# pmgbergen/porepy

Hardware: AMD Instinct MI355X
Metric: cells/sec MPFA assemble+solve, 3D unstructured grid (higher is better)
Workload: dtype f64

## Files before the change

### include/porefv.h

```cpp
#ifndef POREFV_H
#define POREFV_H

#include <stddef.h>
#include <stdint.h>

#ifdef __cplusplus
extern "C" {
#endif

typedef struct pfv_ctx pfv_ctx;

typedef enum {
  PFV_OK = 0,
  PFV_ERR_SINGULAR = 1,
  PFV_ERR_CELL_SHAPE = 2,
  PFV_ERR_HIP = 3,
  PFV_ERR_ARGUMENT = 4,
  PFV_ERR_UNSUPPORTED = 5,
  PFV_ERR_NOT_CONVERGED = 6
} pfv_status;

enum {
  PFV_MAT_FLUX = 0,
  PFV_MAT_BOUND_FLUX = 1,
// ... 128 lines not shown
  double flow_adjoint_map_ms;
  double flow_adjoint_products_ms;
  double flow_adjoint_solve_ms;
  double flow_adjoint_gradient_ms;
  double advdiff_adjoint_ms;
  int64_t advdiff_adjoint_steps;
  int64_t advdiff_adjoint_iterations;
  int64_t advdiff_adjoint_gmres_retries;
  int64_t advdiff_adjoint_precond_fallbacks;
  double advdiff_adjoint_accumulate_ms;
  int64_t flow_adjoint_exact_calls;
  int64_t flow_adjoint_exact_map_builds;
  double flow_adjoint_exact_map_ms;
  double flow_adjoint_exact_ms;
  int64_t spgemm_path;
  int64_t spgemm_lds_bytes;
  double advdiff_adjoint_exact_ms;
  int64_t advdiff_adjoint_exact_passes;
  int64_t advdiff_adjoint_exact_batch;
  double transport_sorb_ms;
  int64_t transport_sorb_steps;
  int64_t transport_sorb_core_iterations;
  int64_t transport_sorb_components;
} pfv_stats;

pfv_status pfv_create(int device, pfv_ctx** out);
void pfv_destroy(pfv_ctx* h);
const char* pfv_last_error(pfv_ctx* h);
int pfv_is_device_build(void);

pfv_status pfv_set_grid(pfv_ctx* h, int nd, int64_t nc, int64_t nf, int64_t nn,
                        const double* nodes, const int32_t* cf_indptr,
                        const int32_t* cf_indices, const int8_t* cf_sign,
                        const int32_t* fn_indptr, const int32_t* fn_indices,
                        const double* face_normals, const double* face_centers,
                        const double* cell_centers, const double* face_areas);

pfv_status pfv_mpfa_set_params(pfv_ctx* h, const double* perm_33n, const uint8_t* bc_flags,
                               const double* robin_weight, double eta,
                               const double* eta_subface);

pfv_status pfv_mpfa_set_permeability(pfv_ctx* h, const double* perm_33n);

#define PFV_AD_WANT_FLUX_JACOBIAN 1u
pfv_status pfv_mpfa_ad_flux_system(pfv_ctx* h, const double* p, const double* dk_dp, const double* bc_values,
                                   const double* vector_source, const double* source, double* flux_out,
// ... 235 lines not shown
pfv_status pfv_csr_divide(pfv_csr* A, double s);
pfv_status pfv_csr_spmv(const pfv_csr* A, const double* x, double* y);
pfv_status pfv_csr_spmv_device(const pfv_csr* A, const double* d_x, double* d_y);
pfv_status pfv_csr_info(const pfv_csr* A, int64_t* nrows, int64_t* ncols, int64_t* nnz);
pfv_status pfv_csr_get(const pfv_csr* A, int32_t* indptr, int32_t* indices, double* values);
pfv_status pfv_csr_set_system(pfv_ctx* h, const pfv_csr* A, const double* rhs, int rhs_on_device);
void pfv_csr_free(pfv_csr* A);

pfv_status pfv_set_stream(pfv_ctx* h, void* hip_stream);
pfv_status pfv_reset_stream(pfv_ctx* h);
pfv_status pfv_sync(pfv_ctx* h);

pfv_status pfv_get_stats(pfv_ctx* h, pfv_stats* out);
pfv_status pfv_get_stats_n(pfv_ctx* h, void* out, size_t struct_size);

enum { PFV_KERNEL_SPMV_A = 0, PFV_KERNEL_NODE = 1, PFV_KERNEL_FACE = 2,
       PFV_KERNEL_AMG_SMOOTH = 3,
       PFV_KERNEL_TRIAD = 4,
       PFV_KERNEL_READ = 5         };
pfv_status pfv_time_kernel(pfv_ctx* h, int kernel, int reps, double* avg_ms);

pfv_status pfv_debug_copy(pfv_ctx* h, int which, double* dst, int64_t count);

#ifdef __cplusplus
}
#endif
#endif
```

### porepy_amd/_lib.py

```python
from __future__ import annotations

import ctypes as C
import os

import numpy as np

_HERE = os.path.dirname(os.path.abspath(__file__))
DEFAULT_LIBRARY = os.path.join(_HERE, "csrc", "libporefv_hip.so")

MAT_FLUX, MAT_BOUND_FLUX, MAT_BOUND_PRESSURE_CELL, MAT_BOUND_PRESSURE_FACE = 0, 1, 2, 3
MAT_VECTOR_SOURCE, MAT_BOUND_PRESSURE_VECTOR_SOURCE, MAT_SYSTEM = 4, 5, 6
MAT_STRESS, MAT_BOUND_STRESS, MAT_BOUND_DISPLACEMENT_CELL, MAT_BOUND_DISPLACEMENT_FACE, MAT_MECH_SYSTEM = 7, 8, 9, 10, 11
MAT_USER_SYSTEM = 12
MAT_FLUX_JACOBIAN = 13
MAT_UPWIND, MAT_UPWIND_RHS_DIR, MAT_UPWIND_RHS_NEU, MAT_TRANSPORT_SYSTEM = 14, 15, 16, 17
MAT_ADVDIFF_SYSTEM = 18
BC_DIR, BC_NEU, BC_ROB, BC_INTERNAL = 1, 2, 4, 8
SOLVE_CG, SOLVE_BICGSTAB, SOLVE_GMRES = 0, 1, 2
PRECOND_JACOBI, PRECOND_AMG, PRECOND_BLOCK, PRECOND_AMG_NNS, PRECOND_SWEEP = 0, 1, 2, 3, 4
FLUXFN_LINEAR, FLUXFN_COREY, FLUXFN_TABLE = 0, 1, 2
ISOTHERM_LINEAR, ISOTHERM_FREUNDLICH, ISOTHERM_LANGMUIR = 0, 1, 2
DISCR_REBUILD_TOPOLOGY, DISCR_SKIP_VECTOR_SOURCE = 1, 2

STATUS_NAMES = {
# ... 2 lines not shown
}

EXPORTS = [
    "pfv_create", "pfv_destroy", "pfv_last_error", "pfv_is_device_build", "pfv_set_grid",
    "pfv_mpfa_set_params", "pfv_mpfa_discretize", "pfv_matrix_info", "pfv_get_matrix",
    "pfv_mpfa_assemble", "pfv_get_rhs", "pfv_spmv", "pfv_solve", "pfv_spmv_device",
    "pfv_get_device_rhs", "pfv_sync", "pfv_get_stats", "pfv_time_kernel", "pfv_debug_copy",
    "pfv_spmv_device_rows", "pfv_copy_device_vector", "pfv_set_stream",
    "pfv_mpsa_set_params", "pfv_mpsa_discretize", "pfv_mpsa_assemble",
    "pfv_mpfa_discretize_faces", "pfv_set_system", "pfv_tpfa_discretize", "pfv_mpsa_discretize_faces", "pfv_set_preconditioner", "pfv_amg_setup", "pfv_amg_setup_sharded", "pfv_amg_apply_device", "pfv_csr_from_host", "pfv_csr_from_matrix", "pfv_csr_block_diag", "pfv_csr_matmul", "pfv_csr_axpby", "pfv_csr_transpose", "pfv_csr_bmat", "pfv_csr_scale", "pfv_csr_divide", "pfv_csr_spmv", "pfv_csr_spmv_device", "pfv_csr_info", "pfv_csr_get", "pfv_csr_set_system", "pfv_csr_free", "pfv_reset_stream", "pfv_mpsa_set_robin", "pfv_mpsa_set_basis", "pfv_mpfa_set_subface_bc", "pfv_mpsa_set_subface_bc", "pfv_mpsa_set_subface_basis",
    "pfv_biot_set_alphas", "pfv_biot_discretize", "pfv_biot_matrix_info", "pfv_biot_get_matrix",
    "pfv_set_vectors_on_device", "pfv_set_periodic", "pfv_biot_discretize_faces", "pfv_solve_sharded", "pfv_tpfa_transmissibility_ad",
    "pfv_get_matrix_rows", "pfv_active_size", "pfv_device_memory",
    "pfv_rccl_unique_id", "pfv_rccl_comm_create", "pfv_rccl_set_halo_plan", "pfv_rccl_hooks", "pfv_rccl_stats",
    "pfv_rccl_last_error", "pfv_rccl_comm_destroy", "pfv_mpfa_ad_flux_system", "pfv_host_alloc", "pfv_host_free",
    "pfv_mpsa_set_subface_eta", "pfv_mpsa_set_reconstruction_eta", "pfv_mpsa_set_reconstruction_eta_subface", "pfv_get_stats_n", "pfv_set_block_preconditioner",
    "pfv_mpfa_set_permeability", "pfv_set_near_null_space", "pfv_amg_nns_level", "pfv_amg_nns_apply_device", "pfv_amg_level",
    "pfv_mpfa_face_flux", "pfv_upwind_set_bc", "pfv_upwind_discretize", "pfv_upwind_assemble", "pfv_transport_advance",
    "pfv_advdiff_assemble", "pfv_advdiff_advance", "pfv_advdiff_face_flux", "pfv_resident_flux",
    "pfv_sweep_info", "pfv_transport_advance_multi", "pfv_transport_advance_nl", "pfv_transport_advance_nl_multi",
    "pfv_transport_advance_react", "pfv_transport_adjoint_multi", "pfv_transport_adjoint_react",
    "pfv_transport_adjoint_nl", "pfv_transport_adjoint_nl_multi", "pfv_flow_adjoint", "pfv_flow_adjoint_exact",
    "pfv_advdiff_adjoint", "pfv_advdiff_adjoint_exact", "pfv_amg_level_rhs", "pfv_transport_advance_sorb",
]


class SolveInfo(C.Structure):
    _fields_ = [("iterations", C.c_int32), ("converged", C.c_int32),
                ("rel_residual", C.c_double), ("solve_ms", C.c_double)]


class Stats(C.Structure):
    _fields_ = [("topology_ms", C.c_double), ("symbolic_ms", C.c_double), ("node_ms", C.c_double),
                ("face_ms", C.c_double), ("assemble_ms", C.c_double), ("solve_ms", C.c_double),
                ("bytes_written_outputs", C.c_double), ("num_nodes", C.c_int64),
                ("num_sub_half_faces", C.c_int64), ("sum_block_sq", C.c_int64),
                ("max_block", C.c_int64), ("amg_setup_ms", C.c_double),
                ("amg_operator_complexity", C.c_double), ("amg_levels", C.c_int64),
                ("amg_coarsest_rows", C.c_int64), ("discretize_ms", C.c_double), ("solve_renumbered", C.c_int64),
                ("node_flops", C.c_double), ("node_table_doubles", C.c_int64),
                ("amg_maps_reused", C.c_int64), ("amg_level0_nnz", C.c_int64), ("amg_filter_theta", C.c_double),
                ("win_reused", C.c_int64), ("amg_filter_layout", C.c_int64),
                ("solve_launches", C.c_int64), ("amg_setup_launches", C.c_int64), ("node_redo", C.c_int64),
                ("symbolic_reused", C.c_int64), ("amg_stale_rematches", C.c_int64),
                ("mpsa_contrast_regions", C.c_int64), ("mpsa_max_contrast", C.c_double), ("assemble_positions_kept", C.c_int64),
                ("pipeline_runs", C.c_int64), ("amg_nns_modes", C.c_int64),
# ... 13 lines not shown
                ("transport_react_ms", C.c_double), ("transport_react_steps", C.c_int64),
                ("transport_react_core_iterations", C.c_int64), ("transport_react_components", C.c_int64),
                ("transport_adjoint_ms", C.c_double), ("transport_adjoint_steps", C.c_int64),
                ("transport_adjoint_core_iterations", C.c_int64), ("amg_ap_nnz", C.c_int64),
                ("transport_react_adjoint_ms", C.c_double), ("transport_react_adjoint_steps", C.c_int64),
                ("transport_react_adjoint_core_iterations", C.c_int64), ("amg_galerkin_ap", C.c_int64),
                ("transport_nl_adjoint_ms", C.c_double), ("transport_nl_adjoint_steps", C.c_int64),
                ("transport_nl_adjoint_core_iterations", C.c_int64),
                ("transport_nlc_adjoint_ms", C.c_double), ("transport_nlc_adjoint_steps", C.c_int64),
                ("transport_nlc_adjoint_core_iterations", C.c_int64),
                ("flow_adjoint_calls", C.c_int64), ("flow_adjoint_iterations", C.c_int64),
                ("flow_adjoint_map_builds", C.c_int64), ("flow_adjoint_map_ms", C.c_double),
                ("flow_adjoint_products_ms", C.c_double), ("flow_adjoint_solve_ms", C.c_double),
                ("flow_adjoint_gradient_ms", C.c_double),
                ("advdiff_adjoint_ms", C.c_double), ("advdiff_adjoint_steps", C.c_int64),
                ("advdiff_adjoint_iterations", C.c_int64), ("advdiff_adjoint_gmres_retries", C.c_int64),
                ("advdiff_adjoint_precond_fallbacks", C.c_int64), ("advdiff_adjoint_accumulate_ms", C.c_double),
                ("flow_adjoint_exact_calls", C.c_int64), ("flow_adjoint_exact_map_builds", C.c_int64),
                ("flow_adjoint_exact_map_ms", C.c_double), ("flow_adjoint_exact_ms", C.c_double),
                ("spgemm_path", C.c_int64), ("spgemm_lds_bytes", C.c_int64),
                ("advdiff_adjoint_exact_ms", C.c_double), ("advdiff_adjoint_exact_passes", C.c_int64),
                ("advdiff_adjoint_exact_batch", C.c_int64),
                ("transport_sorb_ms", C.c_double), ("transport_sorb_steps", C.c_int64),
                ("transport_sorb_core_iterations", C.c_int64), ("transport_sorb_components", C.c_int64)]

    def as_dict(self):
        return {n: getattr(self, n) for n, _ in self._fields_}


HALO_FN = C.CFUNCTYPE(C.c_int, C.c_void_p, C.c_void_p, C.c_void_p)
ALLREDUCE_FN = C.CFUNCTYPE(C.c_int, C.c_void_p, C.c_void_p, C.c_int, C.c_void_p)


SENDRECV_FN = C.CFUNCTYPE(C.c_int, C.c_void_p, C.c_int, C.POINTER(C.c_int32), C.c_void_p, C.POINTER(C.c_int64),
                          C.c_void_p, C.POINTER(C.c_int64), C.c_void_p)
ALLGATHER_FN = C.CFUNCTYPE(C.c_int, C.c_void_p, C.c_void_p, C.c_void_p, C.c_int64, C.c_void_p)


class ShardHooks(C.Structure):
    _fields_ = [("exchange_halo", HALO_FN), ("allreduce_sum", ALLREDUCE_FN), ("user", C.c_void_p),
                ("sendrecv", SENDRECV_FN), ("allgather", ALLGATHER_FN)]


class PorefvError(RuntimeError):
    def __init__(self, status: int, message: str):
        super().__init__(f"porefv status {status} ({STATUS_NAMES.get(status, '?')}): {message}")
        self.status = status
# ... 141 lines not shown
    lib.pfv_rccl_comm_create.restype = C.c_int
    lib.pfv_rccl_set_halo_plan.argtypes = [C.c_void_p, C.c_int, _ip, _i64p, _ip, _i64p, _ip]
    lib.pfv_rccl_set_halo_plan.restype = C.c_int
    lib.pfv_rccl_hooks.argtypes = [C.c_void_p, C.POINTER(ShardHooks)]
    lib.pfv_rccl_hooks.restype = C.c_int
    lib.pfv_rccl_stats.argtypes = [C.c_void_p, _i64p, _i64p, _i64p]
    lib.pfv_rccl_stats.restype = C.c_int
    lib.pfv_rccl_last_error.argtypes = [C.c_void_p]
    lib.pfv_rccl_last_error.restype = C.c_char_p
    lib.pfv_rccl_comm_destroy.argtypes = [C.c_void_p]
    lib.pfv_rccl_comm_destroy.restype = None
    lib.pfv_device_memory.argtypes = [_h, C.POINTER(C.c_int64), C.POINTER(C.c_int64)]
    lib.pfv_device_memory.restype = C.c_int
    lib.pfv_host_alloc.argtypes = [C.c_size_t, C.POINTER(C.c_void_p)]
    lib.pfv_host_alloc.restype = C.c_int
    lib.pfv_host_free.argtypes = [C.c_void_p]
    lib.pfv_host_free.restype = None
    lib.pfv_active_size.argtypes = [_h, C.POINTER(C.c_int64)]
    lib.pfv_active_size.restype = C.c_int
    lib.pfv_get_matrix_rows.argtypes = [_h, C.c_int, C.c_int64, _ip, _ip, _ip, _dp]
    lib.pfv_get_matrix_rows.restype = C.c_int
    lib.pfv_debug_copy.argtypes = [_h, C.c_int, _dp, C.c_int64]
    lib.pfv_debug_copy.restype = C.c_int
    lib.pfv_spmv_device_rows.argtypes = [_h, C.c_int, C.c_int64, C.c_void_p, C.c_void_p]
    lib.pfv_spmv_device_rows.restype = C.c_int
    lib.pfv_copy_device_vector.argtypes = [_h, C.c_int, C.c_void_p, C.c_int64]
    lib.pfv_copy_device_vector.restype = C.c_int
    lib.pfv_tpfa_transmissibility_ad.argtypes = [_h, _dp, _dp, _dp]
    lib.pfv_tpfa_transmissibility_ad.restype = C.c_int
    lib.pfv_solve_sharded.argtypes = [_h, C.c_int, C.c_double, C.c_int, C.c_int64, C.POINTER(ShardHooks),
                                      C.c_void_p, C.c_void_p, C.POINTER(SolveInfo)]
    lib.pfv_solve_sharded.restype = C.c_int
    lib.pfv_set_stream.argtypes = [_h, C.c_void_p]
    lib.pfv_set_stream.restype = C.c_int
    lib.pfv_mpsa_set_params.argtypes = [_h, _dp, _dp, _up, _up, C.c_double]
    lib.pfv_mpsa_set_params.restype = C.c_int
    lib.pfv_mpsa_discretize.argtypes = [_h, C.c_uint32]
    lib.pfv_mpsa_discretize.restype = C.c_int
    lib.pfv_mpsa_assemble.argtypes = [_h, _dp, _dp]
    lib.pfv_mpsa_assemble.restype = C.c_int
    lib.pfv_mpfa_face_flux.argtypes = [_h, _dp, _dp, _dp, _dp]
    lib.pfv_mpfa_face_flux.restype = C.c_int
    lib.pfv_upwind_set_bc.argtypes = [_h, _up]
    lib.pfv_upwind_set_bc.restype = C.c_int
    lib.pfv_upwind_discretize.argtypes = [_h, _dp, C.c_int]
    lib.pfv_upwind_discretize.restype = C.c_int
# ... 1564 lines not shown
               "rel_residual": info.rel_residual, "solve_ms": info.solve_ms}
        return self._adjoint_result(st, grads, out, raise_on_fail)

    def tpfa_transmissibility_ad(self, perm):
        K = _f64(perm)
        if K.shape != (3, 3, self.nc):
            raise ValueError("perm must have shape (3, 3, num_cells)")
        t = np.empty(self.nf, dtype=np.float64)
        jac = np.empty((self.ncf, 9), dtype=np.float64)
        self._check(self.lib.pfv_tpfa_transmissibility_ad(self._h, _ptr(K, _dp), _ptr(t, _dp), _ptr(jac, _dp)))
        return t, jac

    def set_stream(self, stream_ptr: int | None):
        self._check(self.lib.pfv_set_stream(self._h, C.c_void_p(stream_ptr or 0)))

    def reset_stream(self):
        self._check(self.lib.pfv_reset_stream(self._h))

    def debug_array(self, which: int, n: int) -> np.ndarray:
        out = np.empty(n, dtype=np.float64)
        self._check(self.lib.pfv_debug_copy(self._h, int(which), _ptr(out, _dp), n))
        return out

    def time_kernel(self, kernel: int, reps: int = 10) -> float:
        ms = C.c_double()
        self._check(self.lib.pfv_time_kernel(self._h, int(kernel), int(reps), C.byref(ms)))
        return ms.value
```

### porepy_amd/csrc/backend.h

```cpp
#pragma once

#include <algorithm>
#include <atomic>
#include <chrono>
#include <cmath>
#include <cstdint>
#include <cstdio>
#include <cstdlib>
#include <cstring>
#include <numeric>
#include <stdexcept>
#include <string>
#include <type_traits>
#include <unordered_map>
#include <vector>

#ifdef PFV_EMULATE
#define PFV_HD
#define PFV_FN inline
#define PFV_LAMBDA [=]
#else
#include <hip/hip_runtime.h>
#include <rocprim/rocprim.hpp>
#define PFV_HD __host__ __device__
// ... 441 lines not shown
    if (b < n) {
      WaveCtx w{b, pfv_lds + (size_t)grp * lds_per_item, (int)threadIdx.x % G, G, nullptr};
      f(w);
    }
    __syncthreads();
  }
}
#endif

template <class F>
inline void parallel_for(stream_t s, int64_t n, F f) {
  if (n <= 0) return;
#ifdef PFV_EMULATE
  (void)s;
  for (int64_t i = 0; i < n; ++i) f(i);
#else
  int64_t blocks = (n + 255) / 256;
  if (blocks > 16384) blocks = 16384;
  PFV_LAUNCH(HIP_KERNEL_NAME(k_parallel_for<F>), dim3((unsigned)blocks), dim3(256), 0, s, n, f);
  PFV_HIP_CHECK(hipGetLastError());
#endif
}

template <int G = 64, class F>
inline void wave_for(stream_t s, int64_t n, size_t lds_bytes, F f) {
  if (n <= 0) return;
  lds_bytes = (lds_bytes + 15) & ~size_t(15);
#ifdef PFV_EMULATE
  (void)s;
  std::vector<double> lds((lds_bytes + 7) / 8 + 2);
  for (int64_t b = 0; b < n; ++b) {
    WaveCtx w{b, reinterpret_cast<char*>(lds.data()), 0, 1, nullptr};
    f(w);
  }
#else
  constexpr int per_block = 64 / G;
  const size_t block_lds = lds_bytes * per_block;
  if (block_lds > 160 * 1024) throw Error(5, "work item needs more than 160 KiB of LDS");
  int64_t blocks = (n + per_block - 1) / per_block;
  if (blocks > 256 * 64) blocks = 256 * 64;
  if (block_lds > 48 * 1024) {
    PFV_HIP_CHECK(hipFuncSetAttribute(reinterpret_cast<const void*>(&k_wave_for<G, F>),
                                      hipFuncAttributeMaxDynamicSharedMemorySize, (int)block_lds));
  }
  PFV_LAUNCH(HIP_KERNEL_NAME(k_wave_for<G, F>), dim3((unsigned)blocks), dim3(64), block_lds, s, n,
                     lds_bytes, f);
// ... 147 lines not shown

template <class TI, class TO>
inline void exclusive_scan(stream_t s, Scratch& sc, const TI* in, TO* out, size_t n) {
#ifdef PFV_EMULATE
  (void)s; (void)sc;
  TO acc = 0;
  for (size_t i = 0; i < n; ++i) {
    out[i] = acc;
    acc += (TO)in[i];
  }
  out[n] = acc;
#else
  auto it = rocprim::make_transform_iterator(
      rocprim::make_counting_iterator<size_t>(0),
      [in, n] __device__(size_t i) -> TO { return i < n ? (TO)in[i] : TO(0); });
  size_t bytes = 0;
  PFV_HIP_CHECK(rocprim::exclusive_scan(nullptr, bytes, it, out, TO(0), n + 1, rocprim::plus<TO>(), s));
  sc.tmp.ensure(bytes);
  PFV_HIP_CHECK(rocprim::exclusive_scan(sc.tmp.p, bytes, it, out, TO(0), n + 1, rocprim::plus<TO>(), s));
#endif
}

template <class T>
inline T read_scalar(stream_t s, const T* dptr) {
  T v;
  be_d2h(&v, dptr, sizeof(T), s);
  return v;
}

template <class T>
PFV_FN int lower_bound_idx(const T* a, int n, T key) {
  int lo = 0, hi = n;
  while (lo < hi) {
    int mid = (lo + hi) >> 1;
    if (a[mid] < key) lo = mid + 1; else hi = mid;
  }
  return lo;
}

template <class T>
PFV_FN int upper_bound_idx(const T* a, int n, T key) {
  int lo = 0, hi = n;
  while (lo < hi) {
    int mid = (lo + hi) >> 1;
    if (a[mid] <= key) lo = mid + 1; else hi = mid;
  }
// ... 18 lines not shown
}
PFV_HD inline void atomic_max_i32(int* addr, int v) {
#ifdef PFV_EMULATE
  if (v > *addr) *addr = v;
#else
#if defined(__HIP_DEVICE_COMPILE__)
  atomicMax(addr, v);
#else
  (void)addr; (void)v;
#endif
#endif
}
PFV_HD inline void atomic_min_i32(int* addr, int v) {
#ifdef PFV_EMULATE
  if (v < *addr) *addr = v;
#else
#if defined(__HIP_DEVICE_COMPILE__)
  atomicMin(addr, v);
#else
  (void)addr; (void)v;
#endif
#endif
}
PFV_HD inline int atomic_fetch_add_i32(int* addr, int v) {
#ifdef PFV_EMULATE
  const int old = *addr;
  *addr += v;
  return old;
#else
#if defined(__HIP_DEVICE_COMPILE__)
  return atomicAdd(addr, v);
#else
  (void)addr; (void)v;
  return 0;
#endif
#endif
}
PFV_HD inline void atomic_add_i32(int* addr, int v) {
#ifdef PFV_EMULATE
  *addr += v;
#else
#if defined(__HIP_DEVICE_COMPILE__)
  atomicAdd(addr, v);
#else
  (void)addr; (void)v;
#endif
// ... 5 lines not shown
```

### porepy_amd/csrc/ctx.h

```cpp
#pragma once
#include "../../include/porefv.h"
#include "backend.h"

#include <algorithm>
#include <functional>
#include <memory>
#include <vector>

namespace pfv {

constexpr int kMaxFaceNodes = 8;
constexpr int kMaxCellFaces = 16;
constexpr int kMaxBlock = 255;
static const int kClassBounds[] = {4, 8, 12, 16, 24, 32, 40, 48, 64, 96, 128, 192, 255};
constexpr int kNumClasses = 13;

struct alignas(16) SfRec {
  int64_t toff;
  uint8_t n;
  uint8_t ls;
  uint8_t jstar;
  uint8_t deg;
  uint8_t r[3];
  uint8_t pad;
// ... 95 lines not shown
  Buf<int32_t> node_face;
  Buf<int32_t> sf_face;
  Buf<uint8_t> sf_ls;
  Buf<int32_t> face_nsides;
  Buf<int32_t> node_cells;
  Buf<int32_t> node_bptr;
  Buf<int32_t> node_bfaces;
  Buf<uint8_t> node_bls;
  Buf<int64_t> node_tptr;
  Buf<int64_t> node_tbptr;
  Buf<uint8_t> flux_colpairs;
  int64_t cp_stride = 0;
  Buf<uint8_t> node_active;
  Buf<int32_t> face_subset;
  bool biot_rows_complete = false;
  Buf<int32_t> cell_subset;
  Buf<int32_t> face_order;
  double bbox_lo[3] = {0, 0, 0}, bbox_hi[3] = {1, 1, 1};
  Buf<int32_t> node_order;
  std::vector<int64_t> class_begin;
  int max_block = 0, max_deg = 0, max_face_nodes = 0, max_cell_faces = 0, max_bnd_per_node = 0;
  int64_t sum_block_sq = 0;
  int64_t tab_len = 0, tabb_len = 0;

  Buf<double> tab;
  Buf<double> tabb;
  Buf<SfRec> sf_rec;
  Buf<int32_t> face_ctr;
  unsigned face_ctr_next = 0;
  Buf<FaceRec> face_rec;
  Buf<int32_t> status;

  bool have_symbolic = false, have_numeric = false, have_system = false;
  bool have_flow_rhs = false;
  bool rows_complete = false;
  CsrPattern pat_flux, pat_bound, pat_vs, pat_A;
  bool vs_indices_pending = false;
  bool vs_implicit = false;
  Buf<double> val[PFV_NUM_MATS];
  bool filled[PFV_NUM_MATS] = {};
  Buf<double> rhs, diag, xsol, face_tmp, vec_in;
  Buf<double> kry[10];
  Buf<double> red;
  Buf<double> gmres_basis, gmres_small;

  bool have_mpsa_params = false, have_mpsa_numeric = false, have_mpsa_symbolic = false, have_mech_system = false;
// ... 219 lines not shown
```

### porepy_amd/csrc/porefv.hip

```cpp
#include <cmath>
#include <cstring>

#include "ctx.h"
#include "fluxfn.h"
#include "isotherm.h"
#include "react.h"
namespace pfv {
static int rccl_exchange_halo(void* user, double* d_x, void* stream);
}
#include "topology.inc"
#include "mpfa_numeric.inc"
#include "linalg.inc"
#include "reorder.inc"
#include "dd.h"
#include "mpsa.inc"
#include "tpfa.inc"
#include "biot.inc"
#include "ad_flux.inc"
#include "upwind.inc"
#include "advdiff.inc"
#include "sweep.inc"
#include "flow_adjoint.inc"
#include "mpfa_adjoint.inc"
#include "advdiff_adjoint.inc"
// ... 4466 lines not shown
      tm.start(s);
      for (int i = 0; i < reps; ++i) pfv::run_node_kernel(*h);
      *avg_ms = tm.stop(s) / reps;
    } else if (kernel == PFV_KERNEL_FACE) {
      require(h->have_numeric, "discretize first");
      const bool with_vs = h->filled[PFV_MAT_VECTOR_SOURCE];
      tm.start(s);
      for (int i = 0; i < reps; ++i) pfv::run_face_kernel(*h, with_vs);
      *avg_ms = tm.stop(s) / reps;
    } else {
      require(false, "unknown kernel id");
    }
  });
}

pfv_status pfv_debug_copy(pfv_ctx* h, int which, double* dst, int64_t count) {
  return guarded(h, [&] {
    require(h->have_numeric && dst && count >= 0 && count <= (which == 0 ? h->tab_len : h->tabb_len), "bad argument");
    const double* src = which == 0 ? h->tab.p : h->tabb.p;
    be_d2h(dst, src, sizeof(double) * (size_t)count, h->stream);
  });
}

}

#include "rccl_hooks.inc"
#include "csr_algebra.inc"
```

### porepy_amd/csrc/topology.inc

```

namespace pfv {

static void build_topology(pfv_ctx_impl& c) {
  stream_t s = c.stream;
  const int nd = c.nd;
  const int64_t nc = c.nc, nf = c.nf, nn = c.nn, ncf = c.ncf, nsf = c.nsf;
  const int32_t* cf_ptr = c.cf_ptr;
  const int32_t* cf_idx = c.cf_idx;
  const int8_t* cf_sgn = c.cf_sgn;
  const int32_t* fn_ptr = c.fn_ptr;
  const int32_t* fn_idx = c.fn_idx;

  int bits = 1;
  while ((int64_t(1) << bits) < nn + 1 && bits < 32) ++bits;

  Buf<int32_t> cell_of_e, cnt_e;
  Buf<int64_t> h_off;
  cell_of_e.ensure(ncf);
  cnt_e.ensure(ncf + 1);
  h_off.ensure(ncf + 1);
  {
    int32_t* coe = cell_of_e;
    parallel_for(s, nc, PFV_LAMBDA(int64_t cell) {
      for (int e = cf_ptr[cell]; e < cf_ptr[cell + 1]; ++e) coe[e] = (int32_t)cell;
    });
    int32_t* cnt = cnt_e;
// ... 337 lines not shown
      const int n = fp[node + 1] - fp[node];
      int cls = 0;
      while (cls < nclass - 1 && n > bd[cls]) ++cls;
      k[node] = (uint32_t)cls;
      v[node] = (int32_t)node;
    });
    sort_pairs(s, c.scratch, key_in.p, key_out.p, val_in.p, c.node_order.p, (size_t)nn, 4);
    Buf<int32_t> cb_dev;
    int32_t* cbd = cb_dev.ensure(nclass + 1);
    const uint32_t* ks = key_out;
    parallel_for(s, nclass + 1, PFV_LAMBDA(int64_t cls) { cbd[cls] = lower_bound_idx<uint32_t>(ks, (int)nn, (uint32_t)cls); });
    std::vector<int32_t> cbh(nclass + 1);
    be_d2h(cbh.data(), cbd, sizeof(int32_t) * (nclass + 1), s);
    c.class_begin.assign(nclass + 1, nn);
    for (int cls = 0; cls <= nclass; ++cls) c.class_begin[cls] = cbh[cls];
  }
  c.have_topology = true;
  c.topo_key = 0;
  c.stats.num_nodes = nn;
  c.stats.num_sub_half_faces = nh;
  c.stats.sum_block_sq = c.sum_block_sq;
  c.stats.max_block = c.max_block;
  c.stats.node_table_doubles = c.tab_len + c.tabb_len;
}

template <class RankT = uint8_t, int EPL = 4>
PFV_FN int merge_unique_lds(const WaveCtx& w, const int32_t* buf, const int32_t* off, int nl,
                            int32_t* merged, unsigned long long* mask, int32_t* out,
                            RankT* rank_out = nullptr) {
  const int m = off[nl];
  const int nw = (m + 63) >> 6;
  PFV_LANES(i, nw) mask[i] = 0ull;
  for (int e0 = w.lane; e0 < m; e0 += w.width * EPL) {
    int el[EPL], li[EPL], rank[EPL];
    int32_t v[EPL];
#pragma unroll
    for (int u = 0; u < EPL; ++u) {
      const int e = e0 + u * w.width;
      el[u] = e < m ? e : -1;
      const int ee = e < m ? e : 0;
      int l = 0;
      while (l + 1 < nl && ee >= off[l + 1]) ++l;
      li[u] = l;
      v[u] = buf[ee];
      rank[u] = ee - off[l];
    }
// ... 776 lines not shown
```

Measured before the change: 34.77 million.

## Rebuild MPFA topology construction as node-centric pass with fused scans

Adds a new topology builder that constructs per-node sub-half-face tables directly from face-slot arrays. It uses a fused multi-field exclusive scan, per-wave LDS rank sorting, and a single packed device-to-host readback in place of the legacy multi-stage sort pipeline. The aim is to cut kernel launches, global sorts and host syncs during topology setup. If invariants fail (a face with more than two sides, or a node with too many faces), it falls back to the legacy path, which can be forced with an environment variable. A debug export API is also added.

```diff
diff --git a/include/porefv.h b/include/porefv.h
--- a/include/porefv.h
+++ b/include/porefv.h
@@ -174,6 +174,7 @@
   int64_t transport_sorb_steps;
   int64_t transport_sorb_core_iterations;
   int64_t transport_sorb_components;
+  int64_t topology_reference_path;
 } pfv_stats;
 
 pfv_status pfv_create(int device, pfv_ctx** out);
@@ -455,6 +456,8 @@
 
 pfv_status pfv_debug_copy(pfv_ctx* h, int which, double* dst, int64_t count);
 
+pfv_status pfv_debug_topology(pfv_ctx* h, int which, void* dst, int64_t capacity, int64_t* bytes);
+
 #ifdef __cplusplus
 }
 #endif
diff --git a/porepy_amd/_lib.py b/porepy_amd/_lib.py
--- a/porepy_amd/_lib.py
+++ b/porepy_amd/_lib.py
@@ -48,6 +48,7 @@
     "pfv_transport_advance_react", "pfv_transport_adjoint_multi", "pfv_transport_adjoint_react",
     "pfv_transport_adjoint_nl", "pfv_transport_adjoint_nl_multi", "pfv_flow_adjoint", "pfv_flow_adjoint_exact",
     "pfv_advdiff_adjoint", "pfv_advdiff_adjoint_exact", "pfv_amg_level_rhs", "pfv_transport_advance_sorb",
+    "pfv_debug_topology",
 ]
 
 
@@ -107,7 +108,8 @@
                 ("advdiff_adjoint_exact_ms", C.c_double), ("advdiff_adjoint_exact_passes", C.c_int64),
                 ("advdiff_adjoint_exact_batch", C.c_int64),
                 ("transport_sorb_ms", C.c_double), ("transport_sorb_steps", C.c_int64),
-                ("transport_sorb_core_iterations", C.c_int64), ("transport_sorb_components", C.c_int64)]
+                ("transport_sorb_core_iterations", C.c_int64), ("transport_sorb_components", C.c_int64),
+                ("topology_reference_path", C.c_int64)]
 
     def as_dict(self):
         return {n: getattr(self, n) for n, _ in self._fields_}
@@ -295,6 +297,8 @@
     lib.pfv_get_matrix_rows.restype = C.c_int
     lib.pfv_debug_copy.argtypes = [_h, C.c_int, _dp, C.c_int64]
     lib.pfv_debug_copy.restype = C.c_int
+    lib.pfv_debug_topology.argtypes = [_h, C.c_int, C.c_void_p, C.c_int64, _lp]
+    lib.pfv_debug_topology.restype = C.c_int
     lib.pfv_spmv_device_rows.argtypes = [_h, C.c_int, C.c_int64, C.c_void_p, C.c_void_p]
     lib.pfv_spmv_device_rows.restype = C.c_int
     lib.pfv_copy_device_vector.argtypes = [_h, C.c_int, C.c_void_p, C.c_int64]
@@ -1905,6 +1909,31 @@
         self._check(self.lib.pfv_debug_copy(self._h, int(which), _ptr(out, _dp), n))
         return out
 
+    TOPOLOGY_ARRAYS = (
+        ("node_hptr", np.int32), ("h_cell", np.int32), ("h_lf", np.uint8), ("h_sgn", np.int8), ("h_first", np.uint8),
+        ("node_fptr", np.int32), ("node_sf", np.int32), ("sf_face", np.int32), ("sf_ls", np.uint8),
+        ("face_nsides", np.int32), ("node_face", np.int32), ("node_bptr", np.int32), ("node_bfaces", np.int32),
+        ("node_bls", np.uint8), ("node_tptr", np.int64), ("node_tbptr", np.int64), ("node_cells", np.int32),
+        ("face_order", np.int32), ("node_order", np.int32), ("class_begin", np.int64))
+    TOPOLOGY_SCALARS = ("nh", "max_face_nodes", "max_cell_faces", "max_block", "max_deg", "max_bnd_per_node",
+                        "sum_block_sq", "tab_len", "tabb_len", "node_flops_bits", "stats_num_nodes",
+                        "stats_num_sub_half_faces", "stats_sum_block_sq", "stats_max_block",
+                        "stats_node_table_doubles", "topology_digest", "topology_path")
+
+    def debug_topology(self) -> dict:
+        out = {}
+        nbytes = C.c_int64()
+        for which, (name, dtype) in enumerate(self.TOPOLOGY_ARRAYS + (("scalars", np.int64),)):
+            self._check(self.lib.pfv_debug_topology(self._h, which, None, 0, C.byref(nbytes)))
+            arr = np.empty(nbytes.value // np.dtype(dtype).itemsize, dtype=dtype)
+            if arr.size:
+                self._check(self.lib.pfv_debug_topology(self._h, which, arr.ctypes.data_as(C.c_void_p), arr.nbytes,
+                                                        C.byref(nbytes)))
+            out[name] = arr
+        for name, v in zip(self.TOPOLOGY_SCALARS, out.pop("scalars")):
+            out[name] = int(v)
+        return out
+
     def time_kernel(self, kernel: int, reps: int = 10) -> float:
         ms = C.c_double()
         self._check(self.lib.pfv_time_kernel(self._h, int(kernel), int(reps), C.byref(ms)))
diff --git a/porepy_amd/csrc/backend.h b/porepy_amd/csrc/backend.h
--- a/porepy_amd/csrc/backend.h
+++ b/porepy_amd/csrc/backend.h
@@ -487,6 +487,44 @@
 #endif
 }
 
+#ifndef PFV_EMULATE
+template <int NM, class F>
+__global__ void __launch_bounds__(256) k_parallel_for_max(int64_t n, int32_t* out, F f) {
+  __shared__ int32_t red[NM];
+  if ((int)threadIdx.x < NM) red[threadIdx.x] = 0;
+  __syncthreads();
+  int32_t m[NM];
+#pragma unroll
+  for (int k = 0; k < NM; ++k) m[k] = 0;
+  const int64_t stride = (int64_t)gridDim.x * blockDim.x;
+  for (int64_t i = (int64_t)blockIdx.x * blockDim.x + threadIdx.x; i < n; i += stride) f(i, m);
+#pragma unroll
+  for (int k = 0; k < NM; ++k) {
+    if (m[k] > 0) atomicMax(&red[k], m[k]);
+  }
+  __syncthreads();
+  if ((int)threadIdx.x < NM && red[threadIdx.x] > 0) atomicMax(out + threadIdx.x, red[threadIdx.x]);
+}
+#endif
+template <int NM, class F>
+inline void parallel_for_max(stream_t s, int64_t n, int32_t* out, F f) {
+  if (n <= 0) return;
+#ifdef PFV_EMULATE
+  (void)s;
+  int32_t m[NM];
+  for (int k = 0; k < NM; ++k) m[k] = 0;
+  for (int64_t i = 0; i < n; ++i) f(i, m);
+  for (int k = 0; k < NM; ++k) {
+    if (m[k] > out[k]) out[k] = m[k];
+  }
+#else
+  int64_t blocks = (n + 255) / 256;
+  if (blocks > 16384) blocks = 16384;
+  PFV_LAUNCH(HIP_KERNEL_NAME(k_parallel_for_max<NM, F>), dim3((unsigned)blocks), dim3(256), 0, s, n, out, f);
+  PFV_HIP_CHECK(hipGetLastError());
+#endif
+}
+
 template <int G = 64, class F>
 inline void wave_for(stream_t s, int64_t n, size_t lds_bytes, F f) {
   if (n <= 0) return;
@@ -680,6 +718,30 @@
 }
 
 template <class T>
+struct PlusOp {
+  PFV_HD T operator()(const T& a, const T& b) const { return a + b; }
+};
+template <class T, class Gen>
+inline void exclusive_scan_gen(stream_t s, Scratch& sc, Gen gen, T* out, size_t n) {
+#ifdef PFV_EMULATE
+  (void)s; (void)sc;
+  T acc = T();
+  for (size_t i = 0; i < n; ++i) {
+    out[i] = acc;
+    acc = acc + gen((int64_t)i);
+  }
+  out[n] = acc;
+#else
+  auto it = rocprim::make_transform_iterator(rocprim::make_counting_iterator<size_t>(0),
+                                             [gen, n] __device__(size_t i) -> T { return i < n ? gen((int64_t)i) : T(); });
+  size_t bytes = 0;
+  PFV_HIP_CHECK(rocprim::exclusive_scan(nullptr, bytes, it, out, T(), n + 1, PlusOp<T>(), s));
+  sc.tmp.ensure(bytes);
+  PFV_HIP_CHECK(rocprim::exclusive_scan(sc.tmp.p, bytes, it, out, T(), n + 1, PlusOp<T>(), s));
+#endif
+}
+
+template <class T>
 inline T read_scalar(stream_t s, const T* dptr) {
   T v;
   be_d2h(&v, dptr, sizeof(T), s);
@@ -744,6 +806,13 @@
 #endif
 #endif
 }
+PFV_HD inline void store_relaxed_i32(int* addr, int v) {
+#if !defined(PFV_EMULATE) && defined(__HIP_DEVICE_COMPILE__)
+  __hip_atomic_store(addr, v, __ATOMIC_RELAXED, __HIP_MEMORY_SCOPE_AGENT);
+#else
+  *addr = v;
+#endif
+}
 PFV_HD inline int atomic_fetch_add_i32(int* addr, int v) {
 #ifdef PFV_EMULATE
   const int old = *addr;
diff --git a/porepy_amd/csrc/ctx.h b/porepy_amd/csrc/ctx.h
--- a/porepy_amd/csrc/ctx.h
+++ b/porepy_amd/csrc/ctx.h
@@ -141,6 +141,7 @@
   int max_block = 0, max_deg = 0, max_face_nodes = 0, max_cell_faces = 0, max_bnd_per_node = 0;
   int64_t sum_block_sq = 0;
   int64_t tab_len = 0, tabb_len = 0;
+  int topo_path = 0;
 
   Buf<double> tab;
   Buf<double> tabb;
diff --git a/porepy_amd/csrc/porefv.hip b/porepy_amd/csrc/porefv.hip
--- a/porepy_amd/csrc/porefv.hip
+++ b/porepy_amd/csrc/porefv.hip
@@ -4512,6 +4512,59 @@
   });
 }
 
+pfv_status pfv_debug_topology(pfv_ctx* h, int which, void* dst, int64_t capacity, int64_t* bytes) {
+  return guarded(h, [&] {
+    require(h->have_topology && bytes && which >= 0 && which <= 20, "bad argument");
+    auto s = h->stream;
+    const int64_t nn = h->nn, nf = h->nf, nsf = h->nsf, nh = h->nh;
+    const void* src = nullptr;
+    int64_t n = 0;
+    std::vector<int64_t> host;
+    switch (which) {
+      case 0: src = h->node_hptr.p; n = 4 * (nn + 1); break;
+      case 1: src = h->h_cell.p; n = 4 * nh; break;
+      case 2: src = h->h_lf.p; n = nh; break;
+      case 3: src = h->h_sgn.p; n = nh; break;
+      case 4: src = h->h_first.p; n = nh; break;
+      case 5: src = h->node_fptr.p; n = 4 * (nn + 1); break;
+      case 6: src = h->node_sf.p; n = 4 * nsf; break;
+      case 7: src = h->sf_face.p; n = 4 * nsf; break;
+      case 8: src = h->sf_ls.p; n = nsf; break;
+      case 9: src = h->face_nsides.p; n = 4 * nf; break;
+      case 10: src = h->node_face.p; n = 4 * nsf; break;
+      case 11: src = h->node_bptr.p; n = 4 * (nn + 1); break;
+      case 12:
+      case 13: {
+        const int64_t nb = pfv::read_scalar<int32_t>(s, h->node_bptr.p + nn);
+        src = which == 12 ? (const void*)h->node_bfaces.p : (const void*)h->node_bls.p;
+        n = which == 12 ? 4 * nb : nb;
+        break;
+      }
+      case 14: src = h->node_tptr.p; n = 8 * (nn + 1); break;
+      case 15: src = h->node_tbptr.p; n = 8 * (nn + 1); break;
+      case 16: src = h->node_cells.p; n = 4 * (nh / h->nd); break;
+      case 17: src = h->face_order.p; n = 4 * nf; break;
+      case 18: src = h->node_order.p; n = 4 * nn; break;
+      case 19: host.assign(h->class_begin.begin(), h->class_begin.end()); break;
+      default: {
+        int64_t flops_bits = 0;
+        std::memcpy(&flops_bits, &h->stats.node_flops, sizeof(double));
+        host = {nh, h->max_face_nodes, h->max_cell_faces, h->max_block, h->max_deg, h->max_bnd_per_node,
+                h->sum_block_sq, h->tab_len, h->tabb_len, flops_bits, (int64_t)h->stats.num_nodes,
+                (int64_t)h->stats.num_sub_half_faces, (int64_t)h->stats.sum_block_sq, (int64_t)h->stats.max_block,
+                (int64_t)h->stats.node_table_doubles, (int64_t)pfv::topology_digest(*h), (int64_t)h->topo_path};
+        break;
+      }
+    }
+    if (which >= 19) n = 8 * (int64_t)host.size();
+    *bytes = n;
+    if (dst && capacity >= n && n > 0) {
+      if (which >= 19) std::memcpy(dst, host.data(), (size_t)n);
+      else be_d2h(dst, src, (size_t)n, s);
+    }
+  });
+}
+
 }
 
 #include "rccl_hooks.inc"
diff --git a/porepy_amd/csrc/topology.inc b/porepy_amd/csrc/topology.inc
--- a/porepy_amd/csrc/topology.inc
+++ b/porepy_amd/csrc/topology.inc
@@ -1,7 +1,7 @@
 
 namespace pfv {
 
-static void build_topology(pfv_ctx_impl& c) {
+static void build_topology_legacy(pfv_ctx_impl& c) {
   stream_t s = c.stream;
   const int nd = c.nd;
   const int64_t nc = c.nc, nf = c.nf, nn = c.nn, ncf = c.ncf, nsf = c.nsf;
@@ -385,6 +385,390 @@
   c.stats.sum_block_sq = c.sum_block_sq;
   c.stats.max_block = c.max_block;
   c.stats.node_table_doubles = c.tab_len + c.tabb_len;
+}
+
+struct TopoRec {
+  int64_t h, nb, sq, tab, tabb;
+  double fl;
+};
+PFV_HD inline TopoRec operator+(const TopoRec& a, const TopoRec& b) {
+  return TopoRec{a.h + b.h, a.nb + b.nb, a.sq + b.sq, a.tab + b.tab, a.tabb + b.tabb, a.fl + b.fl};
+}
+struct alignas(16) TopoI4 {
+  int32_t x, y, z, w;
+};
+struct TopoClassBounds {
+  int b[kNumClasses];
+};
+constexpr int kTopoKeyCap = 512;
+constexpr int32_t kTopoNoKey = 0x7fffffff;
+
+static bool build_topology_nodes(pfv_ctx_impl& c) {
+  stream_t s = c.stream;
+  const int nd = c.nd;
+  const int64_t nc = c.nc, nf = c.nf, nn = c.nn, ncf = c.ncf, nsf = c.nsf;
+  const int32_t* cf_ptr = c.cf_ptr;
+  const int32_t* cf_idx = c.cf_idx;
+  const int8_t* cf_sgn = c.cf_sgn;
+  const int32_t* fn_ptr = c.fn_ptr;
+  const int32_t* fn_idx = c.fn_idx;
+  const int64_t hcap = 2 * nsf;
+  if (hcap >= (int64_t(1) << 31)) return false;
+
+  int bits = 1;
+  while ((int64_t(1) << bits) < nn + 1 && bits < 32) ++bits;
+
+  Buf<uint32_t> key_in, key_out;
+  Buf<int32_t> val_in, val_out, cell_of_e, face_ends, cnt_n_, nb_n_;
+  const int64_t nkey = std::max(nsf, std::max(nf, nn));
+  key_in.ensure(nkey);
+  key_out.ensure(nkey);
+  val_in.ensure(nkey);
+  int32_t* coe = cell_of_e.ensure(ncf);
+  int32_t* fslot = face_ends.ensure(2 * nf);
+  int32_t* fother = fslot + nf;
+  Buf<int32_t> mx_;
+  int32_t* mx = mx_.ensure(4);
+  int32_t* ns = c.face_nsides.ensure(nf);
+  int32_t* st = c.status.ensure(16);
+  be_memset(fslot, 0xff, sizeof(int32_t) * 2 * nf, s);
+  be_memset(mx, 0, sizeof(int32_t) * 4, s);
+  be_memset(st, 0, sizeof(int32_t) * 16, s);
+
+  c.node_fptr.ensure(nn + 1);
+  c.node_sf.ensure(nsf);
+  c.sf_face.ensure(nsf);
+  c.sf_ls.ensure(nsf);
+  {
+    uint32_t* k = key_in;
+    int32_t* v = val_in;
+    int32_t* sff = c.sf_face;
+    parallel_for(s, nsf, PFV_LAMBDA(int64_t i) {
+      k[i] = (uint32_t)fn_idx[i];
+      v[i] = (int32_t)i;
+    });
+    parallel_for_max<2>(s, std::max(nc, nf), mx, PFV_LAMBDA(int64_t i, int32_t* m) {
+      int fa = 0, fb = 0, ca = 0, cb = 0;
+      if (i < nf) {
+        fa = fn_ptr[i];
+        fb = fn_ptr[i + 1];
+      }
+      if (i < nc) {
+        ca = cf_ptr[i];
+        cb = cf_ptr[i + 1];
+      }
+      int32_t f4[4];
+#pragma unroll
+      for (int u = 0; u < 4; ++u) f4[u] = ca + u < cb ? cf_idx[ca + u] : -1;
+      for (int t = fa; t < fb; ++t) sff[t] = (int32_t)i;
+#pragma unroll
+      for (int u = 0; u < 4; ++u) {
+        if (f4[u] >= 0) {
+          coe[ca + u] = (int32_t)i;
+          store_relaxed_i32(fslot + f4[u], ca + u);
+        }
+      }
+      for (int e = ca + 4; e < cb; ++e) {
+        const int f = cf_idx[e];
+        coe[e] = (int32_t)i;
+        store_relaxed_i32(fslot + f, e);
+      }
+      m[0] = fb - fa > m[0] ? fb - fa : m[0];
+      m[1] = cb - ca > m[1] ? cb - ca : m[1];
+    });
+    parallel_for(s, ncf, PFV_LAMBDA(int64_t e) {
+      const int f = cf_idx[e];
+      if (fslot[f] != (int32_t)e) store_relaxed_i32(fother + f, (int32_t)e);
+    });
+    parallel_for(s, ncf, PFV_LAMBDA(int64_t e) {
+      const int f = cf_idx[e];
+      if (fslot[f] != (int32_t)e && fother[f] != (int32_t)e) atomic_max_i32(mx + 2, 1);
+    });
+  }
+  sort_pairs(s, c.scratch, key_in.p, key_out.p, val_in.p, c.node_sf.p, (size_t)nsf, bits);
+  {
+    int32_t* fp = c.node_fptr;
+    const uint32_t* ks = key_out;
+    parallel_for(s, nn + 1, PFV_LAMBDA(int64_t v) {
+      fp[v] = lower_bound_idx<uint32_t>(ks, (int)nsf, (uint32_t)v);
+    });
+  }
+  int32_t* nm_face = c.node_face.ensure(nsf);
+  int32_t* cnt_n = cnt_n_.ensure(nn);
+  int32_t* nb_n = nb_n_.ensure(nn);
+  {
+    const int32_t* fp = c.node_fptr;
+    const int32_t* nsfp = c.node_sf;
+    const int32_t* sff = c.sf_face;
+    uint8_t* ls = c.sf_ls;
+    wave_for<16>(s, nn, 2 * 16 * sizeof(int32_t), PFV_LAMBDA(const WaveCtx& w) {
+      int32_t* part = reinterpret_cast<int32_t*>(w.lds);
+      const int64_t v = w.item;
+      const int a = fp[v], n = fp[v + 1] - a;
+      int cnt = 0, nb = 0;
+      const bool odd = n > kMaxBlock;
+      PFV_LANES(l, n) {
+        const int sfi = nsfp[a + l];
+        const int f = sff[sfi];
+        const int sides = (fslot[f] >= 0 ? 1 : 0) + (fother[f] >= 0 ? 1 : 0);
+        nm_face[a + l] = f;
+        ls[sfi] = (uint8_t)(l & 0xff);
+        cnt += sides;
+        nb += sides == 1 ? 1 : 0;
+      }
+      if (odd) atomic_max_i32(mx + 2, 1);
+      part[w.lane] = cnt;
+      part[16 + w.lane] = nb;
+      w.lsync();
+      if (w.lane0()) {
+        int tc = 0, tb = 0;
+        for (int i = 0; i < w.width; ++i) {
+          tc += part[i];
+          tb += part[16 + i];
+        }
+        cnt_n[v] = tc;
+        nb_n[v] = tb;
+      }
+      w.lsync();
+    });
+  }
+  Buf<TopoRec> rec_;
+  TopoRec* rec = rec_.ensure(nn + 1);
+  {
+    const int32_t* fp = c.node_fptr;
+    exclusive_scan_gen<TopoRec>(s, c.scratch, PFV_LAMBDA(int64_t v) -> TopoRec {
+      const int n = fp[v + 1] - fp[v], cnt = cnt_n[v], nb = nb_n[v], deg = cnt / nd;
+      TopoRec r;
+      r.h = cnt;
+      r.nb = nb;
+      r.sq = (int64_t)n * n;
+      r.tab = (int64_t)(n + 1) * ((cnt + 1) & ~1);
+      r.tabb = 2 * (int64_t)n * nb;
+      r.fl = 2.0 * n * n * n + 2.0 * nd * n * cnt + 2.0 * (1 + nd) * n * nb + 60.0 * nd * nd * deg;
+      return r;
+    }, rec, (size_t)nn);
+  }
+  c.node_hptr.ensure(nn + 1);
+  c.node_bptr.ensure(nn + 1);
+  c.node_tptr.ensure(nn + 1);
+  c.node_tbptr.ensure(nn + 1);
+  c.h_cell.ensure(hcap);
+  c.h_lf.ensure(hcap);
+  c.h_sgn.ensure(hcap);
+  c.h_first.ensure(hcap);
+  c.node_bfaces.ensure(nsf);
+  c.node_bls.ensure(nsf);
+  c.node_cells.ensure(hcap / nd + 1);
+  {
+    const int32_t* fp = c.node_fptr;
+    int32_t* hp = c.node_hptr;
+    int32_t* bp = c.node_bptr;
+    int64_t* tp = c.node_tptr;
+    int64_t* tbp = c.node_tbptr;
+    int32_t* hc = c.h_cell;
+    uint8_t* lf = c.h_lf;
+    int8_t* hs = c.h_sgn;
+    uint8_t* first = c.h_first;
+    int32_t* bf = c.node_bfaces;
+    uint8_t* bl = c.node_bls;
+    int32_t* ncl = c.node_cells;
+    const size_t lds_bytes = (size_t)kTopoKeyCap * 2 * sizeof(int32_t) + 256;
+    wave_for<64>(s, nn, lds_bytes, PFV_LAMBDA(const WaveCtx& w) {
+      int32_t* keys = reinterpret_cast<int32_t*>(w.lds);
+      int32_t* cellS = keys + kTopoKeyCap;
+      uint8_t* bndL = reinterpret_cast<uint8_t*>(cellS + kTopoKeyCap);
+      const int64_t v = w.item;
+      const int a = fp[v], n = fp[v + 1] - a;
+      const TopoRec r0 = rec[v], r1 = rec[v + 1];
+      const int h0 = (int)r0.h, cnt = (int)(r1.h - r0.h), b0 = (int)r0.nb, nb = (int)(r1.nb - r0.nb);
+      if (w.lane0()) {
+        hp[v] = h0;
+        bp[v] = b0;
+        tp[v] = r0.tab;
+        tbp[v] = r0.tabb;
+        if (v == nn - 1) {
+          hp[nn] = (int32_t)r1.h;
+          bp[nn] = (int32_t)r1.nb;
+          tp[nn] = r1.tab;
+          tbp[nn] = r1.tabb;
+        }
+        track_max_i32(st + 1, n);
+        track_max_i32(st + 2, cnt / nd);
+        track_max_i32(st + 3, nb);
+        if (cnt % nd) atomic_max_i32(st + 0, 2);
+      }
+      if (n <= kMaxBlock) {
+        PFV_LANES(l, n) {
+          const int f = nm_face[a + l];
+          const int32_t e0 = fslot[f], e1 = fother[f];
+          keys[l] = e0 < 0 ? kTopoNoKey : (e1 < 0 || e0 < e1 ? e0 : e1);
+          keys[n + l] = e1 < 0 ? kTopoNoKey : (e0 < e1 ? e1 : e0);
+          bndL[l] = (e0 >= 0 && e1 < 0) ? 1 : 0;
+        }
+        PFV_LANES(t, (4 - ((2 * n) & 3)) & 3) keys[2 * n + t] = kTopoNoKey;
+        w.lsync();
+        const int n4 = (2 * n + 3) >> 2;
+        const TopoI4* k4 = reinterpret_cast<const TopoI4*>(keys);
+        PFV_LANES(l, n) {
+          const int32_t k0 = keys[l], k1 = keys[n + l];
+          const bool s0 = k0 != kTopoNoKey, s1 = k1 != kTopoNoKey;
+          const int32_t c0 = s0 ? coe[k0] : -1, c1 = s1 ? coe[k1] : -1;
+          const int8_t g0 = s0 ? cf_sgn[k0] : (int8_t)0, g1 = s1 ? cf_sgn[k1] : (int8_t)0;
+          int q0 = 0, q1 = 0;
+          for (int u = 0; u < n4; ++u) {
+            const TopoI4 q = k4[u];
+            q0 += (q.x < k0 ? 1 : 0) + (q.y < k0 ? 1 : 0) + (q.z < k0 ? 1 : 0) + (q.w < k0 ? 1 : 0);
+            q1 += (q.x < k1 ? 1 : 0) + (q.y < k1 ? 1 : 0) + (q.z < k1 ? 1 : 0) + (q.w < k1 ? 1 : 0);
+          }
+          if (s0) {
+            cellS[q0] = c0;
+            lf[h0 + q0] = (uint8_t)l;
+            first[h0 + q0] = 1;
+            hs[h0 + q0] = g0;
+          }
+          if (s1) {
+            cellS[q1] = c1;
+            lf[h0 + q1] = (uint8_t)l;
+            first[h0 + q1] = c1 == c0 ? 1 : 0;
+            hs[h0 + q1] = g1;
+          }
+        }
+        w.lsync();
+        PFV_LANES(p, cnt) {
+          const int32_t cc = cellS[p];
+          hc[h0 + p] = cc;
+          const bool bad = (p % nd) ? (cc != cellS[p - 1]) : (p > 0 && cc <= cellS[p - 1]);
+          if (bad) atomic_max_i32(st + 0, 2);
+          if (p % nd == 0) ncl[(h0 + p) / nd] = cc;
+        }
+        if (nb > 0) {
+          PFV_LANES(l, n) {
+            if (bndL[l]) {
+              int o = b0;
+              for (int t = 0; t < l; ++t) o += bndL[t];
+              bf[o] = nm_face[a + l];
+              bl[o] = (uint8_t)l;
+            }
+          }
+        }
+      }
+      w.lsync();
+    });
+  }
+
+  c.face_order.ensure(nf);
+  {
+    uint32_t* k = key_in;
+    int32_t* v = val_in;
+    const double* fc = c.fcen;
+    double lo[3], sc[3];
+    for (int d = 0; d < 3; ++d) {
+      lo[d] = c.bbox_lo[d];
+      const double ext = c.bbox_hi[d] - c.bbox_lo[d];
+      sc[d] = ext > 0 ? 1023.999 / ext : 0.0;
+    }
+    const double lo0 = lo[0], lo1 = lo[1], lo2 = lo[2], sc0 = sc[0], sc1 = sc[1], sc2 = sc[2];
+    parallel_for(s, nf, PFV_LAMBDA(int64_t f) {
+      uint32_t q[3];
+      q[0] = (uint32_t)((fc[f] - lo0) * sc0);
+      q[1] = (uint32_t)((fc[nf + f] - lo1) * sc1);
+      q[2] = (uint32_t)((fc[2 * nf + f] - lo2) * sc2);
+      uint32_t code = 0;
+      for (int d = 0; d < 3; ++d) {
+        uint32_t x = q[d] & 0x3ffu;
+        x = (x | (x << 16)) & 0x030000ffu;
+        x = (x | (x << 8)) & 0x0300f00fu;
+        x = (x | (x << 4)) & 0x030c30c3u;
+        x = (x | (x << 2)) & 0x09249249u;
+        code |= x << d;
+      }
+      k[f] = code;
+      v[f] = (int32_t)f;
+      ns[f] = (fslot[f] >= 0 ? 1 : 0) + (fother[f] >= 0 ? 1 : 0);
+    });
+    sort_pairs(s, c.scratch, key_in.p, key_out.p, val_in.p, c.face_order.p, (size_t)nf, 30);
+  }
+  constexpr int nclass = kNumClasses;
+  constexpr int kPack = 13;
+  Buf<int64_t> pack_;
+  int64_t* pk = pack_.ensure(kPack + nclass + 1);
+  {
+    TopoClassBounds bd;
+    for (int i = 0; i < nclass; ++i) bd.b[i] = kClassBounds[i];
+    uint32_t* k = key_in;
+    int32_t* v = val_in;
+    c.node_order.ensure(nn);
+    const int32_t* fp = c.node_fptr;
+    parallel_for(s, nn, PFV_LAMBDA(int64_t node) {
+      const int n = fp[node + 1] - fp[node];
+      int cls = 0;
+      while (cls < nclass - 1 && n > bd.b[cls]) ++cls;
+      k[node] = (uint32_t)cls;
+      v[node] = (int32_t)node;
+    });
+    sort_pairs(s, c.scratch, key_in.p, key_out.p, val_in.p, c.node_order.p, (size_t)nn, 4);
+    const uint32_t* ks = key_out;
+    parallel_for(s, nclass + 2, PFV_LAMBDA(int64_t t) {
+      if (t <= nclass) {
+        pk[kPack + t] = lower_bound_idx<uint32_t>(ks, (int)nn, (uint32_t)t);
+      } else {
+        const TopoRec tot = rec[nn];
+        pk[0] = tot.h;
+        pk[1] = tot.nb;
+        pk[2] = tot.sq;
+        pk[3] = tot.tab;
+        pk[4] = tot.tabb;
+        reinterpret_cast<double*>(pk)[5] = tot.fl;
+        for (int i = 0; i < 4; ++i) pk[6 + i] = st[i];
+        pk[10] = mx[2];
+        pk[11] = mx[0];
+        pk[12] = mx[1];
+      }
+    });
+  }
+  int64_t ph[kPack + nclass + 1];
+  be_d2h(ph, pk, sizeof(ph), s);
+  if (ph[10] != 0) return false;
+  const int64_t nh = ph[0];
+  if (nh >= (int64_t(1) << 31)) throw Error(5, "more than 2^31 sub-half-faces on one device");
+  c.nh = nh;
+  c.max_face_nodes = (int)ph[11];
+  if (c.max_face_nodes > kMaxFaceNodes)
+    throw Error(PFV_ERR_UNSUPPORTED, "faces with more than 8 nodes are not supported");
+  c.max_cell_faces = (int)ph[12];
+  if (c.max_cell_faces > kMaxCellFaces)
+    throw Error(PFV_ERR_UNSUPPORTED, "cells with more than 16 faces are not supported");
+  if (ph[6] == 2)
+    throw Error(PFV_ERR_CELL_SHAPE,
+                "a cell does not have exactly nd faces meeting in one of its nodes (e.g. pyramid)");
+  c.max_block = (int)ph[7];
+  c.max_deg = (int)ph[8];
+  c.max_bnd_per_node = (int)ph[9];
+  if (c.max_block > kMaxBlock || c.max_deg > kMaxBlock)
+    throw Error(PFV_ERR_UNSUPPORTED, "more than 255 faces or cells meet in one node");
+  c.sum_block_sq = ph[2];
+  std::memcpy(&c.stats.node_flops, &ph[5], sizeof(double));
+  c.tab_len = ph[3];
+  c.tabb_len = ph[4];
+  c.class_begin.assign(nclass + 1, nn);
+  for (int cls = 0; cls <= nclass; ++cls) c.class_begin[cls] = ph[kPack + cls];
+  c.have_topology = true;
+  c.topo_key = 0;
+  c.stats.num_nodes = nn;
+  c.stats.num_sub_half_faces = nh;
+  c.stats.sum_block_sq = c.sum_block_sq;
+  c.stats.max_block = c.max_block;
+  c.stats.node_table_doubles = c.tab_len + c.tabb_len;
+  return true;
+}
+
+static void build_topology(pfv_ctx_impl& c) {
+  c.topo_path = 1;
+  if (env_int("PFV_TOPO_LEGACY", 0) != 0 || !build_topology_nodes(c)) {
+    c.topo_path = 0;
+    build_topology_legacy(c);
+  }
+  c.stats.topology_reference_path = c.topo_path == 0 ? 1 : 0;
 }
 
 template <class RankT = uint8_t, int EPL = 4>
```

Result: faster. 35.71 million, median of 6 (+2.7%).
